# bwittmann/transoar

Hardware: AMD Instinct MI355X
Metric: training-step CT volumes/s, 160x160x256 Focused-Decoder (higher is better)
Workload: dtype bf16

## Files before the change

transoar_amd/_build.py:

```python
import os
import subprocess
import sys
from concurrent.futures import ThreadPoolExecutor

PKG = os.path.dirname(os.path.abspath(__file__))
CSRC = os.path.join(PKG, "csrc")
HIPCC = os.environ.get("HIPCC", "/opt/rocm/bin/hipcc")
COMMON_FLAGS = ["--offload-arch=gfx950", "-O3", "-std=c++17", "-shared", "-fPIC",
                "-munsafe-fp-atomics", "-Wall", "-Wno-unused-function"]

LIBS = {
    "libtransoar_msda3d.so": ["msda3d.hip", "msda3d_sort.hip"],
    "libtransoar_conv3d.so": ["conv3d.hip"],
    "libtransoar_instnorm.so": ["instnorm.hip"],
    "libtransoar_rows.so": ["rows.hip"],
    "libtransoar_tokens.so": ["tokens.hip"],
    "libtransoar_gemm.so": ["gemm.hip", "gemm_stream.hip"],
    "libtransoar_convgemm.so": ["conv_gemm.hip"],
    "libtransoar_attn.so": ["attn.hip"],
    "libtransoar_optim.so": ["optim.hip"],
    "libtransoar_criterion.so": ["criterion.hip"],
    "libtransoar_segproxy.so": ["seg_proxy.hip"],
}


def lib_path(name):
    return os.path.join(PKG, name)


def _dep_path(name):
    return os.path.join(PKG, "." + name + ".d")


def _deps(name):
    try:
        if len(LIBS[name]) != 1:
            raise OSError("no depfile for a library of several sources")
        with open(_dep_path(name)) as f:
            words = f.read().replace("\\\n", " ").split()
        deps = [w for w in words[1:] if not w.startswith("/opt/") and not w.startswith("/usr/")]
        if deps:
            return deps + [os.path.join(CSRC, s) for s in LIBS[name]]
    except OSError:
        pass
    inc = os.path.join(PKG, "..", "include")
    return [os.path.join(CSRC, f) for f in os.listdir(CSRC)] + [os.path.join(inc, f) for f in os.listdir(inc)]


def is_stale(name):
    out = lib_path(name)
    if not os.path.exists(out):
        return True
    t = os.path.getmtime(out)
    for d in _deps(name):
        try:
            if os.path.getmtime(d) > t:
                return True
        except OSError:
            return True
    return False


def _compile(name, verbose):
    cmd = [HIPCC] + COMMON_FLAGS + [os.path.join(CSRC, s) for s in LIBS[name]] + ["-o", lib_path(name)]
    if len(LIBS[name]) == 1:
        cmd += ["-MD", "-MF", _dep_path(name)]
    elif os.path.exists(_dep_path(name)):
        os.remove(_dep_path(name))
    if verbose:
        print("[transoar_amd] " + " ".join(cmd), file=sys.stderr)
    subprocess.check_call(cmd)
    return name


def build(force=False, verbose=True, only=None):
    names = [n for n in LIBS if (only is None or n in only) and (force or is_stale(n))]
    if not names:
        return []
    with ThreadPoolExecutor(max_workers=min(len(names), os.cpu_count() or 4)) as pool:
        return list(pool.map(lambda n: _compile(n, verbose), names))


if __name__ == "__main__":
    build(force="--force" in sys.argv)
```

transoar_amd/shadow.py:

```python
import torch
import torch.nn.functional as F

from . import rows

_ALIGN = 64
_current = None


class ShadowWeights:
    def __init__(self, model, stacks=()):
        params = [p for p in model.parameters() if p.dtype == torch.float32 and p.is_contiguous() and p.numel() > 0]
        if not params or len({p.device for p in params}) != 1:
            raise ValueError("ShadowWeights: needs fp32 parameters on one device")
        self.device = params[0].device
        known = {id(p) for p in params}
        order, placed, self._stacks = [], set(), {}
        for group in stacks:
            group = tuple(group)
            if all(id(p) in known and id(p) not in placed for p in group) and \
                    all(p.numel() % 8 == 0 for p in group[:-1]) and len({tuple(p.shape[1:]) for p in group}) == 1:
                order.append(group)
                placed.update(id(p) for p in group)
        order += [(p,) for p in params if id(p) not in placed]
        total, offsets = 0, []
        for group in order:
            total = -(-total // _ALIGN) * _ALIGN
            offsets.append(total)
            total += sum(p.numel() for p in group)
        self.flat = torch.empty(total, dtype=torch.bfloat16, device=self.device)
        alias = torch.empty(0, dtype=torch.bfloat16, device=self.device).set_(self.flat.untyped_storage(), 0, self.flat.shape)
        self.params, self.views, self._writers, self._index = [], [], [], {}
        for group, off in zip(order, offsets):
            start = off
            for p in group:
                v = self.flat[off: off + p.numel()].view(p.shape)
                self.params.append(p)
                self.views.append(v)
                self._writers.append(alias[off: off + p.numel()].view(p.shape))
                self._index[id(p)] = v
                off += p.numel()
            if len(group) > 1:
                rows = sum(p.shape[0] for p in group)
                self._stacks[tuple(id(p) for p in group)] = self.flat[start: off].view(rows, *group[0].shape[1:])
        self._ptrs = [p.data_ptr() for p in self.params]
        self.generation, self._versions = 0, None

    def valid(self):
        return all(p.data_ptr() == q and p.dtype == torch.float32 for p, q in zip(self.params, self._ptrs))

    def refresh(self):
        versions = tuple(p._version for p in self.params)
        if versions != self._versions:
            self.generation += 1
            self._versions = versions
        with torch.no_grad():
            torch._foreach_copy_(self._writers, self.params)

    def get(self, p):
        v = self._index.get(id(p))
        if v is None and getattr(p, "_base", None) is not None and p.is_contiguous():
            base = self._index.get(id(p._base))
            if base is not None and p.numel() == base.numel() and p.storage_offset() == p._base.storage_offset():
                v = base.view(p.shape)
        return v

    def get_stack(self, group):
        return self._stacks.get(tuple(id(p) for p in group))


class fresh:

    def __init__(self, registry):
        self.registry = registry

    def __enter__(self):
        global _current
        self._prev, _current = _current, self.registry
        return self.registry

    def __exit__(self, *exc):
        global _current
        _current = self._prev
        return False


def stamp(ctx):
    ctx._shadow_stamp = None if _current is None else (_current, _current.generation)


def check(ctx):
    st = getattr(ctx, "_shadow_stamp", None)
    if st is not None and st[0].generation != st[1]:
        raise RuntimeError("transoar_amd.shadow: the bf16 weight mirrors were refreshed with changed weights between this "
                           "forward and its backward (two graphs kept alive across an optimizer step / weight load): the "
                           "backward would use the new weights.  Run backward before the next step's forward.")


def bf16(p):
    return None if _current is None else _current.get(p)


def bf16_or_cast(p):
    v = bf16(p)
    return p.to(torch.bfloat16) if v is None else v


def bf16_stack(group):
    return None if _current is None else _current.get_stack(group)


class _Linear(torch.autograd.Function):

    @staticmethod
    def forward(ctx, x, weight, bias, wb, bb):
        xb = x if x.dtype == torch.bfloat16 else x.to(torch.bfloat16)
        ctx.save_for_backward(xb, wb)
        stamp(ctx)
        ctx.in_dtype, ctx.has_bias = x.dtype, bias is not None
        with torch.autocast("cuda", enabled=False):
            return F.linear(xb, wb, bb)

    @staticmethod
    def backward(ctx, gy):
        check(ctx)
        xb, wb = ctx.saved_tensors
        gx = gw = gb = None
        with torch.autocast("cuda", enabled=False):
            gy2 = gy.reshape(-1, gy.shape[-1])
            if gy2.dtype != torch.bfloat16:
                gy2 = gy2.to(torch.bfloat16)
            if ctx.needs_input_grad[0]:
                gx = (gy2 @ wb).view(xb.shape)
                if gx.dtype != ctx.in_dtype:
                    gx = gx.to(ctx.in_dtype)
            if ctx.needs_input_grad[1]:
                gw = torch.mm(gy2.t(), xb.reshape(-1, xb.shape[-1]), out_dtype=torch.float32)
            if ctx.has_bias and ctx.needs_input_grad[2]:
                gb = rows.colsum_any(gy2)
        return gx, gw, gb, None, None


def linear(x, weight, bias=None):
    wb = bf16(weight)
    if wb is None or not x.is_cuda or not torch.is_autocast_enabled() or x.dtype not in (torch.float32, torch.bfloat16):
        return F.linear(x, weight, bias)
    bb = None if bias is None else bf16(bias)
    if bias is not None and bb is None:
        return F.linear(x, weight, bias)
    return _Linear.apply(x, weight, bias, wb, bb)


class _AsBf16(torch.autograd.Function):

    @staticmethod
    def forward(ctx, param):
        return bf16(param).detach()

    @staticmethod
    def backward(ctx, g):
        return g.float()


def as_bf16(p):
    m = bf16(p)
    return p.to(torch.bfloat16) if m is None else _AsBf16.apply(p)


def as_dtype(p, dtype):
    return as_bf16(p) if dtype == torch.bfloat16 else p.to(dtype)


class _SelfAttnProj(torch.autograd.Function):

    @staticmethod
    def forward(ctx, x_qk, x_v, weight, bias, wb, bb):
        c = weight.shape[1]
        xq = x_qk if x_qk.dtype == torch.bfloat16 else x_qk.to(torch.bfloat16)
        xv = x_v if x_v.dtype == torch.bfloat16 else x_v.to(torch.bfloat16)
        ctx.save_for_backward(xq, xv, wb)
        stamp(ctx)
        ctx.dtypes = (x_qk.dtype, x_v.dtype)
        with torch.autocast("cuda", enabled=False):
            return F.linear(xq, wb[:2 * c], bb[:2 * c]), F.linear(xv, wb[2 * c:], bb[2 * c:])

    @staticmethod
    def backward(ctx, g_qk, g_v):
        check(ctx)
        xq, xv, wb = ctx.saved_tensors
        c = wb.shape[1]
        with torch.autocast("cuda", enabled=False):
            g1 = g_qk.reshape(-1, 2 * c).to(torch.bfloat16)
            g2 = g_v.reshape(-1, c).to(torch.bfloat16)
            gxq = (g1 @ wb[:2 * c]).view(xq.shape).to(ctx.dtypes[0]) if ctx.needs_input_grad[0] else None
            gxv = (g2 @ wb[2 * c:]).view(xv.shape).to(ctx.dtypes[1]) if ctx.needs_input_grad[1] else None
            gw = torch.cat((torch.mm(g1.t(), xq.reshape(-1, c), out_dtype=torch.float32),
                            torch.mm(g2.t(), xv.reshape(-1, c), out_dtype=torch.float32)))
            gb = torch.cat((rows.colsum_any(g1), rows.colsum_any(g2)))
        return gxq, gxv, gw, gb, None, None


def self_attention(mha, x_qk, x_v):
    if not (isinstance(mha, torch.nn.MultiheadAttention) and mha._qkv_same_embed_dim and mha.in_proj_bias is not None
            and mha.bias_k is None and not mha.add_zero_attn and x_qk.is_cuda and torch.is_autocast_enabled()):
        return None
    wb, bb = bf16(mha.in_proj_weight), bf16(mha.in_proj_bias)
    if wb is None or bb is None or bf16(mha.out_proj.weight) is None:
        return None
    b, q, c = x_qk.shape
    h = mha.num_heads
    qk, v = _SelfAttnProj.apply(x_qk, x_v, mha.in_proj_weight, mha.in_proj_bias, wb, bb)
    qk = qk.view(b, q, 2, h, c // h)
    out = F.scaled_dot_product_attention(qk[:, :, 0].transpose(1, 2), qk[:, :, 1].transpose(1, 2),
                                         v.view(b, q, h, c // h).transpose(1, 2),
                                         dropout_p=mha.dropout if mha.training else 0.0)
    return linear(out.transpose(1, 2).reshape(b, q, c), mha.out_proj.weight, mha.out_proj.bias)
```

Baseline: 64.37.

## Add fused MFMA self-attention kernel for head dim 48 in decoder

Adds a custom HIP flash-style self-attention forward and backward kernel for head dimension 48 and up to 576 tokens. It stages K/V into swizzled LDS, computes scores with MFMA, and generates dropout masks in-kernel with a hash. The decoder self-attention path is routed to it in place of PyTorch SDPA, which removes layout transposes and generic kernel overhead. The trade-offs are a hash-based dropout RNG instead of PyTorch's and a forward that recomputes scores in two passes.

Result: no change. 64.90, median of 6 (+0.8%).

```diff
diff --git a/include/transoar_selfattn.h b/include/transoar_selfattn.h
--- /dev/null
+++ b/include/transoar_selfattn.h
@@ -0,0 +1,28 @@
+#ifndef TRANSOAR_SELFATTN_H
+#define TRANSOAR_SELFATTN_H
+#ifdef __cplusplus
+extern "C" {
+#endif
+
+enum {
+  TRANSOAR_SELFATTN_OK = 0,
+  TRANSOAR_SELFATTN_ERR_NULL = -1,
+  TRANSOAR_SELFATTN_ERR_DIM = -2,
+  TRANSOAR_SELFATTN_ERR_ALIGN = -3
+};
+
+int transoar_self_attn_forward(const void* qk, const void* v, void* out, float* lse, int B, int S, int H, int D,
+                               float scale, const int* seed, float keep_prob, void* hip_stream);
+
+int transoar_self_attn_backward(const void* qk, const void* v, const void* out, const void* dout, const float* lse,
+                                void* dqk, void* dv, int B, int S, int H, int D, float scale, const int* seed,
+                                float keep_prob, void* hip_stream);
+
+int transoar_selfattn_abi_version(void);
+
+int transoar_self_attn_max_tokens(int D);
+
+#ifdef __cplusplus
+}
+#endif
+#endif
diff --git a/transoar_amd/_build.py b/transoar_amd/_build.py
--- a/transoar_amd/_build.py
+++ b/transoar_amd/_build.py
@@ -21,6 +21,7 @@
     "libtransoar_optim.so": ["optim.hip"],
     "libtransoar_criterion.so": ["criterion.hip"],
     "libtransoar_segproxy.so": ["seg_proxy.hip"],
+    "libtransoar_selfattn.so": ["self_attn.hip"],
 }
 
 
diff --git a/transoar_amd/csrc/self_attn.hip b/transoar_amd/csrc/self_attn.hip
--- /dev/null
+++ b/transoar_amd/csrc/self_attn.hip
@@ -0,0 +1,398 @@
+#include <hip/hip_runtime.h>
+#include <stdint.h>
+
+#include "../../include/transoar_selfattn.h"
+
+#include "mfma_stream.hpp"
+
+namespace transoar {
+
+constexpr int kSaD = 48;
+constexpr int kSaPieces = kSaD / 8;
+constexpr int kSaPitch = 128;
+constexpr int kSaMaxS = 576;
+constexpr int kSaTileBytes = kSaMaxS * kSaPitch;
+constexpr int kSaLds = 2 * kSaTileBytes + 2 * kSaMaxS * 4;
+
+__device__ __forceinline__ int sa_off(int row, int piece) {
+  const int key = (((row >> 1) & 1) << 2) | ((row >> 2) & 3);
+  return row * kSaPitch + ((piece ^ key) << 4);
+}
+__device__ __forceinline__ s16x8 sa_rows(const unsigned char* tile, int lane, int r0, int ks) {
+  return *reinterpret_cast<const s16x8*>(tile + sa_off(r0 + (lane & 31), 2 * ks + (lane >> 5)));
+}
+__device__ __forceinline__ s16x8 sa_cols(const unsigned char* tile, int lane, int R0, int ct) {
+  const int kh = lane >> 5, r = (lane & 15) >> 2, g = (lane >> 4) & 1, c = lane & 3;
+  const int n0 = R0 + 8 * kh + r, n1 = n0 + 4;
+  const int p = 4 * ct + 2 * g + (c >> 1);
+  const s16x4 b0 = __builtin_amdgcn_ds_read_tr16_b64_v4i16((lds_s16x4*)(tile + sa_off(n0, p) + 8 * (c & 1)));
+  const s16x4 b1 = __builtin_amdgcn_ds_read_tr16_b64_v4i16((lds_s16x4*)(tile + sa_off(n1, p) + 8 * (c & 1)));
+  return __builtin_shufflevector(b0, b1, 0, 1, 2, 3, 4, 5, 6, 7);
+}
+__device__ __forceinline__ void sa_stage2(unsigned char* t0, const unsigned short* __restrict__ s0, long stride0, unsigned char* t1,
+                                          const unsigned short* __restrict__ s1, long stride1, int S, int n_tiles) {
+  const int total = n_tiles * 32 * kSaPieces;
+#pragma unroll 4
+  for (int idx = threadIdx.x; idx < total; idx += 256) {
+    const int row = idx / kSaPieces, piece = idx - row * kSaPieces;
+    u32x4 a{0u, 0u, 0u, 0u}, b{0u, 0u, 0u, 0u};
+    if (row < S) {
+      a = *reinterpret_cast<const u32x4*>(s0 + row * stride0 + 8 * piece);
+      b = *reinterpret_cast<const u32x4*>(s1 + row * stride1 + 8 * piece);
+    }
+    *reinterpret_cast<u32x4*>(t0 + sa_off(row, piece)) = a;
+    *reinterpret_cast<u32x4*>(t1 + sa_off(row, piece)) = b;
+  }
+}
+__device__ __forceinline__ void sa_row_frags(const unsigned short* __restrict__ row_ptr, bool ok, int kh, s16x8 (&f)[3]) {
+#pragma unroll
+  for (int ks = 0; ks < 3; ++ks) {
+    u32x4 x{0u, 0u, 0u, 0u};
+    if (ok) x = *reinterpret_cast<const u32x4*>(row_ptr + 16 * ks + 8 * kh);
+    f[ks] = __builtin_bit_cast(s16x8, x);
+  }
+}
+
+struct SaDrop {
+  unsigned seed, thr16;
+  bool on, even;
+};
+__device__ __forceinline__ unsigned sa_hash32(unsigned x) {
+  x ^= x >> 16; x *= 0x7feb352du; x ^= x >> 15; x *= 0x846ca68bu; x ^= x >> 16;
+  return x;
+}
+__device__ __forceinline__ bool sa_keep1(const SaDrop& d, unsigned e) {
+  const unsigned h = sa_hash32((e >> 1) * 0x9e3779b9u + d.seed);
+  return ((e & 1u) ? (h >> 16) : (h & 0xffffu)) < d.thr16;
+}
+__device__ __forceinline__ unsigned sa_keep4(const SaDrop& d, unsigned e0) {
+  if (d.even) {
+    const unsigned h0 = sa_hash32((e0 >> 1) * 0x9e3779b9u + d.seed), h1 = sa_hash32(((e0 >> 1) + 1u) * 0x9e3779b9u + d.seed);
+    return ((h0 & 0xffffu) < d.thr16 ? 1u : 0u) | ((h0 >> 16) < d.thr16 ? 2u : 0u) | ((h1 & 0xffffu) < d.thr16 ? 4u : 0u) |
+           ((h1 >> 16) < d.thr16 ? 8u : 0u);
+  }
+  unsigned bits = 0u;
+#pragma unroll
+  for (unsigned x = 0; x < 4; ++x) bits |= sa_keep1(d, e0 + x) ? (1u << x) : 0u;
+  return bits;
+}
+
+__device__ __forceinline__ void sa_store(unsigned short* __restrict__ dst, const f32x16 (&acc)[2], int kh, float mul) {
+#pragma unroll
+  for (int ct = 0; ct < 2; ++ct)
+#pragma unroll
+    for (int qd = 0; qd < (ct == 0 ? 4 : 2); ++qd)
+      *reinterpret_cast<u32x2*>(dst + 32 * ct + 8 * qd + 4 * kh) =
+          u32x2{pack_bf16(acc[ct][4 * qd] * mul, acc[ct][4 * qd + 1] * mul), pack_bf16(acc[ct][4 * qd + 2] * mul, acc[ct][4 * qd + 3] * mul)};
+}
+
+__device__ __forceinline__ f32x16 sa_scores(const unsigned char* kt, int lane, int t, const s16x8 (&qf)[3], int S) {
+  f32x16 sT;
+#pragma unroll
+  for (int r = 0; r < 16; ++r) sT[r] = 0.f;
+#pragma unroll
+  for (int ks = 0; ks < 3; ++ks) sT = mfma(sa_rows(kt, lane, 32 * t, ks), qf[ks], sT);
+  if (32 * t + 32 > S) {
+    const int kh = lane >> 5;
+#pragma unroll
+    for (int r = 0; r < 16; ++r)
+      if (32 * t + (r & 3) + 8 * (r >> 2) + 4 * kh >= S) sT[r] = -INFINITY;
+  }
+  return sT;
+}
+
+__global__ __launch_bounds__(256) void self_attn_fwd(const unsigned short* __restrict__ qk, const unsigned short* __restrict__ v,
+                                                     unsigned short* __restrict__ out, float* __restrict__ lse2, const int* __restrict__ seed,
+                                                     int S, int H, float scale2, unsigned thr16, float inv_keep) {
+  __shared__ __attribute__((aligned(16))) unsigned char lds[2 * kSaTileBytes];
+  unsigned char* kt = lds;
+  unsigned char* vt = lds + kSaTileBytes;
+  const int lane = threadIdx.x & 63, wave = uniform(threadIdx.x >> 6);
+  const int kh = lane >> 5;
+  const int bh = blockIdx.y, b = bh / H, h = bh - b * H;
+  const int n_tiles = (S + 31) >> 5;
+  const long tok_qk = 2L * H * kSaD, tok_v = static_cast<long>(H) * kSaD;
+  const unsigned short* q0 = qk + static_cast<long>(b) * S * tok_qk + h * kSaD;
+  const unsigned short* v0 = v + static_cast<long>(b) * S * tok_v + h * kSaD;
+  const int row0 = blockIdx.x * 128 + wave * 32;
+  const int i = row0 + (lane & 31);
+  const bool row_ok = i < S;
+  SaDrop drop;
+  drop.on = thr16 < 65536u;
+  drop.seed = drop.on ? static_cast<unsigned>(*seed) : 0u;
+  drop.thr16 = thr16;
+  drop.even = (S & 1) == 0;
+
+  s16x8 qf[3];
+  sa_row_frags(q0 + i * tok_qk, row_ok, kh, qf);
+  sa_stage2(kt, q0 + H * kSaD, tok_qk, vt, v0, tok_v, S, n_tiles);
+  __syncthreads();
+  if (row0 >= S) return;
+
+  float m_run = -INFINITY, l_run = 0.f;
+  for (int t = 0; t < n_tiles; ++t) {
+    const f32x16 sT = sa_scores(kt, lane, t, qf, S);
+    float mt = m_run;
+#pragma unroll
+    for (int r = 0; r < 16; ++r) mt = fmaxf(mt, sT[r] * scale2);
+    const float m_use = mt == -INFINITY ? 0.f : mt;
+    l_run *= fast_exp2(m_run - m_use);
+#pragma unroll
+    for (int r = 0; r < 16; ++r) l_run += fast_exp2(__builtin_fmaf(sT[r], scale2, -m_use));
+    m_run = mt;
+  }
+  const float m_o = other_half(m_run), l_o = other_half(l_run);
+  const float m2 = fmaxf(m_run, m_o);
+  const float l = l_run * fast_exp2(m_run - m2) + l_o * fast_exp2(m_o - m2);
+
+  f32x16 acc[2];
+#pragma unroll
+  for (int ct = 0; ct < 2; ++ct)
+#pragma unroll
+    for (int r = 0; r < 16; ++r) acc[ct][r] = 0.f;
+  const unsigned rowbase = (static_cast<unsigned>(bh) * S + min(i, S - 1)) * S;
+  for (int t = 0; t < n_tiles; ++t) {
+    const f32x16 sT = sa_scores(kt, lane, t, qf, S);
+    float p[16];
+#pragma unroll
+    for (int r = 0; r < 16; ++r) p[r] = fast_exp2(__builtin_fmaf(sT[r], scale2, -m2));
+    if (drop.on) {
+#pragma unroll
+      for (int qd = 0; qd < 4; ++qd) {
+        const unsigned bits = sa_keep4(drop, rowbase + 32 * t + 8 * qd + 4 * kh);
+#pragma unroll
+        for (int e = 0; e < 4; ++e)
+          if (!((bits >> e) & 1u)) p[4 * qd + e] = 0.f;
+      }
+    }
+    s16x8 pf[2];
+    column_to_b_frags(p, pf);
+#pragma unroll
+    for (int j = 0; j < 2; ++j)
+#pragma unroll
+      for (int ct = 0; ct < 2; ++ct) acc[ct] = mfma(sa_cols(vt, lane, 32 * t + 16 * j, ct), pf[j], acc[ct]);
+  }
+  if (row_ok) {
+    sa_store(out + (static_cast<long>(b) * S + i) * tok_v + h * kSaD, acc, kh, inv_keep / l);
+    if (kh == 0) lse2[static_cast<long>(bh) * S + i] = m2 + log2f(l);
+  }
+}
+
+__global__ __launch_bounds__(256) void self_attn_bwd(const unsigned short* __restrict__ qk, const unsigned short* __restrict__ v,
+                                                     const unsigned short* __restrict__ out, const unsigned short* __restrict__ dout,
+                                                     const float* __restrict__ lse2, unsigned short* __restrict__ dqk,
+                                                     unsigned short* __restrict__ dv, const int* __restrict__ seed, int S, int H,
+                                                     int n_blk, float scale, unsigned thr16, float inv_keep) {
+  __shared__ __attribute__((aligned(16))) unsigned char lds[kSaLds];
+  const int lane = threadIdx.x & 63, wave = uniform(threadIdx.x >> 6);
+  const int kh = lane >> 5;
+  const int bh = blockIdx.y, b = bh / H, h = bh - b * H;
+  const int n_tiles = (S + 31) >> 5;
+  const long tok_qk = 2L * H * kSaD, tok_v = static_cast<long>(H) * kSaD;
+  const unsigned short* q0 = qk + static_cast<long>(b) * S * tok_qk + h * kSaD;
+  const unsigned short* k0 = q0 + H * kSaD;
+  const unsigned short* v0 = v + static_cast<long>(b) * S * tok_v + h * kSaD;
+  const unsigned short* o0 = out + static_cast<long>(b) * S * tok_v + h * kSaD;
+  const unsigned short* d0 = dout + static_cast<long>(b) * S * tok_v + h * kSaD;
+  const float scale2 = scale * kLog2e;
+  SaDrop drop;
+  drop.on = thr16 < 65536u;
+  drop.seed = drop.on ? static_cast<unsigned>(*seed) : 0u;
+  drop.thr16 = thr16;
+  drop.even = (S & 1) == 0;
+  const unsigned headbase = static_cast<unsigned>(bh) * S;
+
+  if (static_cast<int>(blockIdx.x) >= n_blk) {
+    unsigned char* kt = lds;
+    unsigned char* vt = lds + kSaTileBytes;
+    const int row0 = (blockIdx.x - n_blk) * 128 + wave * 32;
+    const int i = row0 + (lane & 31);
+    const bool row_ok = i < S;
+    s16x8 qf[3], df[3];
+    sa_row_frags(q0 + i * tok_qk, row_ok, kh, qf);
+    sa_row_frags(d0 + i * tok_v, row_ok, kh, df);
+    float dpart = 0.f;
+#pragma unroll
+    for (int ks = 0; ks < 3; ++ks) {
+      u32x4 o4{0u, 0u, 0u, 0u};
+      if (row_ok) o4 = *reinterpret_cast<const u32x4*>(o0 + i * tok_v + 16 * ks + 8 * kh);
+      const u32x4 d4 = __builtin_bit_cast(u32x4, df[ks]);
+#pragma unroll
+      for (int e = 0; e < 4; ++e) dpart += bf16_lo(o4[e]) * bf16_lo(d4[e]) + bf16_hi(o4[e]) * bf16_hi(d4[e]);
+    }
+    const float lse_i = row_ok ? lse2[static_cast<long>(bh) * S + i] : INFINITY;
+    sa_stage2(kt, k0, tok_qk, vt, v0, tok_v, S, n_tiles);
+    const float dsum = dpart + other_half(dpart);
+    __syncthreads();
+    if (row0 >= S) return;
+
+    f32x16 dq[2];
+#pragma unroll
+    for (int ct = 0; ct < 2; ++ct)
+#pragma unroll
+      for (int r = 0; r < 16; ++r) dq[ct][r] = 0.f;
+    const unsigned rowbase = (headbase + min(i, S - 1)) * S;
+    for (int t = 0; t < n_tiles; ++t) {
+      const f32x16 sT = sa_scores(kt, lane, t, qf, S);
+      f32x16 dpT;
+#pragma unroll
+      for (int r = 0; r < 16; ++r) dpT[r] = 0.f;
+#pragma unroll
+      for (int ks = 0; ks < 3; ++ks) dpT = mfma(sa_rows(vt, lane, 32 * t, ks), df[ks], dpT);
+      unsigned dpk[8];
+#pragma unroll
+      for (int qd = 0; qd < 4; ++qd) {
+        const unsigned bits = drop.on ? sa_keep4(drop, rowbase + 32 * t + 8 * qd + 4 * kh) : 0xfu;
+        float ds[4];
+#pragma unroll
+        for (int e = 0; e < 4; ++e) {
+          const int r = 4 * qd + e;
+          const float pr = fast_exp2(__builtin_fmaf(sT[r], scale2, -lse_i));
+          const float dp = ((bits >> e) & 1u) ? dpT[r] * inv_keep : 0.f;
+          ds[e] = pr * (dp - dsum) * scale;
+        }
+        dpk[2 * qd] = pack_bf16(ds[0], ds[1]);
+        dpk[2 * qd + 1] = pack_bf16(ds[2], ds[3]);
+      }
+      s16x8 dsf[2];
+      packed_column_to_b_frags(dpk, dsf);
+#pragma unroll
+      for (int j = 0; j < 2; ++j)
+#pragma unroll
+        for (int ct = 0; ct < 2; ++ct) dq[ct] = mfma(sa_cols(kt, lane, 32 * t + 16 * j, ct), dsf[j], dq[ct]);
+    }
+    if (row_ok) sa_store(dqk + (static_cast<long>(b) * S + i) * tok_qk + h * kSaD, dq, kh, 1.f);
+    return;
+  }
+
+  unsigned char* qt = lds;
+  unsigned char* dt = lds + kSaTileBytes;
+  float* st_lse = reinterpret_cast<float*>(lds + 2 * kSaTileBytes);
+  float* st_dsum = st_lse + kSaMaxS;
+  const int key0 = blockIdx.x * 128 + wave * 32;
+  const int key = key0 + (lane & 31);
+  const bool key_ok = key < S;
+  s16x8 kf[3], vf[3];
+  sa_row_frags(k0 + key * tok_qk, key_ok, kh, kf);
+  sa_row_frags(v0 + key * tok_v, key_ok, kh, vf);
+  for (int r = threadIdx.x; r < n_tiles * 32; r += 256) {
+    float ls = INFINITY, dsum = 0.f;
+    if (r < S) {
+      ls = lse2[static_cast<long>(bh) * S + r];
+#pragma unroll
+      for (int pc = 0; pc < kSaPieces; ++pc) {
+        const u32x4 o4 = *reinterpret_cast<const u32x4*>(o0 + r * tok_v + 8 * pc);
+        const u32x4 d4 = *reinterpret_cast<const u32x4*>(d0 + r * tok_v + 8 * pc);
+#pragma unroll
+        for (int e = 0; e < 4; ++e) dsum += bf16_lo(o4[e]) * bf16_lo(d4[e]) + bf16_hi(o4[e]) * bf16_hi(d4[e]);
+      }
+    }
+    st_lse[r] = ls;
+    st_dsum[r] = dsum;
+  }
+  sa_stage2(qt, q0, tok_qk, dt, d0, tok_v, S, n_tiles);
+  __syncthreads();
+  if (key0 >= S) return;
+
+  f32x16 gv[2], gk[2];
+#pragma unroll
+  for (int ct = 0; ct < 2; ++ct)
+#pragma unroll
+    for (int r = 0; r < 16; ++r) { gv[ct][r] = 0.f; gk[ct][r] = 0.f; }
+  const unsigned keyc = static_cast<unsigned>(min(key, S - 1));
+  for (int rt = 0; rt < n_tiles; ++rt) {
+    f32x16 s, dp;
+#pragma unroll
+    for (int r = 0; r < 16; ++r) { s[r] = 0.f; dp[r] = 0.f; }
+#pragma unroll
+    for (int ks = 0; ks < 3; ++ks) {
+      s = mfma(sa_rows(qt, lane, 32 * rt, ks), kf[ks], s);
+      dp = mfma(sa_rows(dt, lane, 32 * rt, ks), vf[ks], dp);
+    }
+    unsigned ppk[8], dpk[8];
+#pragma unroll
+    for (int qd = 0; qd < 4; ++qd) {
+      const int rw = 32 * rt + 8 * qd + 4 * kh;
+      const float4 l4 = *reinterpret_cast<const float4*>(st_lse + rw);
+      const float4 d4 = *reinterpret_cast<const float4*>(st_dsum + rw);
+      const float ls[4] = {l4.x, l4.y, l4.z, l4.w}, dd[4] = {d4.x, d4.y, d4.z, d4.w};
+      float pr[4], dsr[4];
+#pragma unroll
+      for (int e = 0; e < 4; ++e) {
+        const int r = 4 * qd + e;
+        const float p = key_ok ? fast_exp2(__builtin_fmaf(s[r], scale2, -ls[e])) : 0.f;
+        const bool keep = !drop.on || sa_keep1(drop, (headbase + static_cast<unsigned>(rw + e)) * S + keyc);
+        pr[e] = keep ? p * inv_keep : 0.f;
+        dsr[e] = p * ((keep ? dp[r] * inv_keep : 0.f) - dd[e]) * scale;
+      }
+      ppk[2 * qd] = pack_bf16(pr[0], pr[1]); ppk[2 * qd + 1] = pack_bf16(pr[2], pr[3]);
+      dpk[2 * qd] = pack_bf16(dsr[0], dsr[1]); dpk[2 * qd + 1] = pack_bf16(dsr[2], dsr[3]);
+    }
+    s16x8 pf[2], dsf[2];
+    packed_column_to_b_frags(ppk, pf);
+    packed_column_to_b_frags(dpk, dsf);
+#pragma unroll
+    for (int j = 0; j < 2; ++j)
+#pragma unroll
+      for (int ct = 0; ct < 2; ++ct) {
+        gv[ct] = mfma(sa_cols(dt, lane, 32 * rt + 16 * j, ct), pf[j], gv[ct]);
+        gk[ct] = mfma(sa_cols(qt, lane, 32 * rt + 16 * j, ct), dsf[j], gk[ct]);
+      }
+  }
+  if (key_ok) {
+    sa_store(dqk + (static_cast<long>(b) * S + key) * tok_qk + (H + h) * kSaD, gk, kh, 1.f);
+    sa_store(dv + (static_cast<long>(b) * S + key) * tok_v + h * kSaD, gv, kh, 1.f);
+  }
+}
+
+}
+
+using namespace transoar;
+
+static bool misaligned(const void* p) { return (reinterpret_cast<uintptr_t>(p) & 15u) != 0; }
+
+static int check_dims(int B, int S, int H, int D, float scale, float keep_prob) {
+  if (D != kSaD || S < 1 || S > kSaMaxS || B < 1 || H < 1 || !(scale > 0.f) || !(keep_prob > 0.f)) return TRANSOAR_SELFATTN_ERR_DIM;
+  const long bh = static_cast<long>(B) * H;
+  if (bh > 65535 || bh * S * S >= (1L << 32)) return TRANSOAR_SELFATTN_ERR_DIM;
+  return TRANSOAR_SELFATTN_OK;
+}
+static unsigned threshold16(float keep_prob) {
+  if (keep_prob >= 1.f) return 65536u;
+  const int t = static_cast<int>(keep_prob * 65536.0f + 0.5f);
+  return static_cast<unsigned>(t < 0 ? 0 : (t > 65535 ? 65535 : t));
+}
+
+extern "C" int transoar_self_attn_forward(const void* qk, const void* v, void* out, float* lse, int B, int S, int H, int D, float scale,
+                                          const int* seed, float keep_prob, void* hip_stream) {
+  if (!qk || !v || !out || !lse || (keep_prob < 1.f && !seed)) return TRANSOAR_SELFATTN_ERR_NULL;
+  const int rc = check_dims(B, S, H, D, scale, keep_prob);
+  if (rc != TRANSOAR_SELFATTN_OK) return rc;
+  if (misaligned(qk) || misaligned(v) || misaligned(out) || misaligned(lse)) return TRANSOAR_SELFATTN_ERR_ALIGN;
+  const float inv_keep = keep_prob >= 1.f ? 1.f : 1.f / keep_prob;
+  hipLaunchKernelGGL(self_attn_fwd, dim3((S + 127) / 128, B * H), dim3(256), 0, static_cast<hipStream_t>(hip_stream),
+                     static_cast<const unsigned short*>(qk), static_cast<const unsigned short*>(v), static_cast<unsigned short*>(out), lse,
+                     seed, S, H, scale * kLog2e, threshold16(keep_prob), inv_keep);
+  return static_cast<int>(hipGetLastError());
+}
+
+extern "C" int transoar_self_attn_backward(const void* qk, const void* v, const void* out, const void* dout, const float* lse, void* dqk,
+                                           void* dv, int B, int S, int H, int D, float scale, const int* seed, float keep_prob,
+                                           void* hip_stream) {
+  if (!qk || !v || !out || !dout || !lse || !dqk || !dv || (keep_prob < 1.f && !seed)) return TRANSOAR_SELFATTN_ERR_NULL;
+  const int rc = check_dims(B, S, H, D, scale, keep_prob);
+  if (rc != TRANSOAR_SELFATTN_OK) return rc;
+  if (misaligned(qk) || misaligned(v) || misaligned(out) || misaligned(dout) || misaligned(lse) || misaligned(dqk) || misaligned(dv))
+    return TRANSOAR_SELFATTN_ERR_ALIGN;
+  const float inv_keep = keep_prob >= 1.f ? 1.f : 1.f / keep_prob;
+  const int n_blk = (S + 127) / 128;
+  hipLaunchKernelGGL(self_attn_bwd, dim3(2 * n_blk, B * H), dim3(256), 0, static_cast<hipStream_t>(hip_stream),
+                     static_cast<const unsigned short*>(qk), static_cast<const unsigned short*>(v), static_cast<const unsigned short*>(out),
+                     static_cast<const unsigned short*>(dout), lse, static_cast<unsigned short*>(dqk), static_cast<unsigned short*>(dv), seed,
+                     S, H, n_blk, scale, threshold16(keep_prob), inv_keep);
+  return static_cast<int>(hipGetLastError());
+}
+
+extern "C" int transoar_selfattn_abi_version(void) { return 1; }
+
+extern "C" int transoar_self_attn_max_tokens(int D) { return D == kSaD ? kSaMaxS : 0; }
diff --git a/transoar_amd/self_attn.py b/transoar_amd/self_attn.py
--- /dev/null
+++ b/transoar_amd/self_attn.py
@@ -0,0 +1,90 @@
+import ctypes
+import os
+
+import torch
+
+from . import _native, tokens
+
+_LIB_PATH = os.path.join(os.path.dirname(os.path.abspath(__file__)), "libtransoar_selfattn.so")
+ABI_VERSION = 1
+HEAD_DIM = 48
+
+
+def _load():
+    if not os.path.exists(_LIB_PATH):
+        raise _native.NativeLibraryError("%s is not built (python transoar_amd/_build.py)" % _LIB_PATH)
+    lib = ctypes.CDLL(_LIB_PATH)
+    i, p, f = ctypes.c_int, ctypes.c_void_p, ctypes.c_float
+    lib.transoar_self_attn_forward.restype = i
+    lib.transoar_self_attn_forward.argtypes = [p, p, p, p, i, i, i, i, f, p, f, p]
+    lib.transoar_self_attn_backward.restype = i
+    lib.transoar_self_attn_backward.argtypes = [p, p, p, p, p, p, p, i, i, i, i, f, p, f, p]
+    lib.transoar_self_attn_max_tokens.restype = i
+    lib.transoar_self_attn_max_tokens.argtypes = [i]
+    lib.transoar_selfattn_abi_version.restype = i
+    if lib.transoar_selfattn_abi_version() != ABI_VERSION:
+        raise _native.NativeLibraryError("%s: ABI mismatch, rebuild" % _LIB_PATH)
+    return lib
+
+
+lib = _load()
+MAX_TOKENS = lib.transoar_self_attn_max_tokens(HEAD_DIM)
+ENABLED = os.environ.get("TRANSOAR_FD_SELF_ATTN", "1") != "0"
+
+
+def _check(rc, what):
+    if rc != 0:
+        raise RuntimeError("%s failed with code %d" % (what, rc))
+
+
+def _stream():
+    return torch.cuda.current_stream().cuda_stream
+
+
+def usable(qk, v, heads, p):
+    return (ENABLED and qk.is_cuda and v.is_cuda and qk.dtype == torch.bfloat16 and v.dtype == torch.bfloat16
+            and v.dim() == 3 and qk.is_contiguous() and v.is_contiguous() and v.shape[2] == heads * HEAD_DIM
+            and qk.numel() == 2 * v.numel() and qk.shape[:2] == v.shape[:2] and 1 <= v.shape[1] <= MAX_TOKENS
+            and v.shape[0] >= 1 and 0.0 <= p < 1.0)
+
+
+class _SelfAttention(torch.autograd.Function):
+    @staticmethod
+    def forward(ctx, qk, v, seed, heads, scale, keep_prob):
+        b, s, c = v.shape
+        out = torch.empty((b, s, c), dtype=torch.bfloat16, device=v.device)
+        lse2 = torch.empty((b, heads, s), dtype=torch.float32, device=v.device)
+        with torch.cuda.device(v.device):
+            _check(lib.transoar_self_attn_forward(qk.data_ptr(), v.data_ptr(), out.data_ptr(), lse2.data_ptr(), b, s, heads, c // heads,
+                                                  float(scale), None if seed is None else seed.data_ptr(), float(keep_prob), _stream()),
+                   "transoar_self_attn_forward")
+        ctx.save_for_backward(qk, v, out, lse2, seed)
+        ctx.heads, ctx.scale, ctx.keep_prob = heads, float(scale), float(keep_prob)
+        return out
+
+    @staticmethod
+    def backward(ctx, dout):
+        qk, v, out, lse2, seed = ctx.saved_tensors
+        b, s, c = v.shape
+        dout = dout.to(torch.bfloat16).contiguous()
+        dqk = torch.empty_like(qk)
+        dv = torch.empty_like(v)
+        with torch.cuda.device(v.device):
+            _check(lib.transoar_self_attn_backward(qk.data_ptr(), v.data_ptr(), out.data_ptr(), dout.data_ptr(), lse2.data_ptr(),
+                                                   dqk.data_ptr(), dv.data_ptr(), b, s, ctx.heads, c // ctx.heads, ctx.scale,
+                                                   None if seed is None else seed.data_ptr(), ctx.keep_prob, _stream()),
+                   "transoar_self_attn_backward")
+        return dqk, dv, None, None, None, None
+
+
+def self_attention(qk, v, heads, p=0.0, seed=None, scale=None):
+    keep_prob = 1.0 - float(p)
+    if keep_prob >= 1.0:
+        seed = None
+    elif seed is None:
+        seed = tokens.dropout_seed(v)
+    else:
+        seed = seed.detach().to(torch.int32).reshape(1).clone()
+    if scale is None:
+        scale = HEAD_DIM ** -0.5
+    return _SelfAttention.apply(qk, v, seed, heads, scale, keep_prob)
diff --git a/transoar_amd/shadow.py b/transoar_amd/shadow.py
--- a/transoar_amd/shadow.py
+++ b/transoar_amd/shadow.py
@@ -1,7 +1,7 @@
 import torch
 import torch.nn.functional as F
 
-from . import rows
+from . import rows, self_attn
 
 _ALIGN = 64
 _current = None
@@ -204,11 +204,22 @@
             and mha.bias_k is None and not mha.add_zero_attn and x_qk.is_cuda and torch.is_autocast_enabled()):
         return None
     wb, bb = bf16(mha.in_proj_weight), bf16(mha.in_proj_bias)
-    if wb is None or bb is None or bf16(mha.out_proj.weight) is None:
-        return None
     b, q, c = x_qk.shape
     h = mha.num_heads
+    if wb is None or bb is None or bf16(mha.out_proj.weight) is None:
+        p = mha.dropout if mha.training else 0.0
+        if not (self_attn.ENABLED and torch.get_autocast_dtype("cuda") == torch.bfloat16 and x_v.shape == x_qk.shape
+                and c == h * self_attn.HEAD_DIM and 1 <= q <= self_attn.MAX_TOKENS and 0.0 <= p < 1.0):
+            return None
+        w, bias = mha.in_proj_weight, mha.in_proj_bias
+        qk, v = F.linear(x_qk, w[:2 * c], bias[:2 * c]), F.linear(x_v, w[2 * c:], bias[2 * c:])
+        if not self_attn.usable(qk, v, h, p):
+            return None
+        return F.linear(self_attn.self_attention(qk, v, h, p), mha.out_proj.weight, mha.out_proj.bias)
     qk, v = _SelfAttnProj.apply(x_qk, x_v, mha.in_proj_weight, mha.in_proj_bias, wb, bb)
+    p = mha.dropout if mha.training else 0.0
+    if self_attn.usable(qk, v, h, p):
+        return linear(self_attn.self_attention(qk, v, h, p), mha.out_proj.weight, mha.out_proj.bias)
     qk = qk.view(b, q, 2, h, c // h)
     out = F.scaled_dot_product_attention(qk[:, :, 0].transpose(1, 2), qk[:, :, 1].transpose(1, 2),
                                          v.view(b, q, h, c // h).transpose(1, 2),
```
